# alphanumericslab/EpidemicModeling

Hardware: AMD Instinct MI355X
Metric: region-day EKF steps/sec (300 regions x 400 days x 250 costs) (higher is better)
Workload: dtype f64; 1 GPU; cfg4: SIAlphaModelEKFOptControlled sweep, 300 regions x 250 cost weights x (400+120) days; chains_per_gpu=75000, days=520, outputs=all, storage=f64, spinup_passes=14, lane_block=40, sweep_chains_total=75000, region_day_steps_per_pass_per_gpu=39000000, historic_only_steps_per_pass_per_gpu=30000000, scoring_tail=True

## Files before the change

epidemicmodeling_amd/_build.py:

```python
from __future__ import annotations

import os
import shutil
import subprocess

HERE = os.path.dirname(os.path.abspath(__file__))
SRC = os.path.join(HERE, "csrc", "epiekf.hip")
DEPS = [SRC, os.path.join(HERE, "csrc", "launch_plan.hpp"), os.path.join(HERE, "csrc", "ekf_device.hpp"), os.path.join(HERE, "csrc", "ekf_sym.hpp"), os.path.join(HERE, "csrc", "ekf_quad.hpp"), os.path.join(HERE, "csrc", "ekf_wave.hpp"), os.path.join(HERE, "csrc", "ekf_hex.hpp"), os.path.join(HERE, "csrc", "ekf_lane6.hpp"),
        os.path.join(HERE, "csrc", "scenario_kernels.hpp"), os.path.join(HERE, "csrc", "rt_expfit.hpp"), os.path.join(HERE, "csrc", "preprocess.hpp"), os.path.join(HERE, "csrc", "nnls.hpp"), os.path.join(HERE, "csrc", "lookahead.hpp"), os.path.join(HERE, "csrc", "rt_window.hpp"), os.path.join(HERE, "csrc", "lasso.hpp"), os.path.join(HERE, "csrc", "ens_summary.hpp"), os.path.join(HERE, "csrc", "ens_score.hpp"), os.path.join(HERE, "csrc", "path_functionals.hpp"), os.path.join(HERE, "csrc", "ar_forecast.hpp"), os.path.join(HERE, "csrc", "two_filter.hpp"), os.path.join(HERE, "csrc", "robust_fit.hpp"), os.path.join(HERE, "csrc", "rate_map.hpp"), os.path.join(HERE, "csrc", "mldivide.hpp"), os.path.join(HERE, "csrc", "svr.hpp"), os.path.join(HERE, "csrc", "loglik.hpp"), os.path.join(HERE, "csrc", "npi_plan.hpp"), os.path.join(HERE, "csrc", "smoother_draws.hpp"), os.path.join(HERE, "csrc", "host_stage.hpp"),
        os.path.join(HERE, "..", "include", "epiekf.h"), os.path.join(HERE, "..", "include", "epiekf_layout.h")]
LIB = os.path.join(HERE, "libepiekf.so")

HIPCC_FLAGS = ["--offload-arch=gfx950", "-O3", "-std=c++17", "-ffp-contract=off", "-fPIC", "-shared"]


def source_hash() -> str:
    import hashlib
    h = hashlib.sha256()
    for d in sorted(DEPS):
        h.update(os.path.basename(d).encode())
        h.update(open(d, "rb").read())
    return h.hexdigest()[:16]


def hipcc() -> str:
    for cand in (shutil.which("hipcc"), "/opt/rocm/bin/hipcc"):
        if cand and os.path.exists(cand):
            return cand
    raise RuntimeError("hipcc not found: libepiekf.so cannot be built")


def is_stale() -> bool:
    if not os.path.exists(LIB):
        return True
    t = os.path.getmtime(LIB)
    return any(os.path.getmtime(d) > t for d in DEPS)


def build_library(force: bool = False, verbose: bool = False) -> str:
    if force or is_stale():
        cmd = [hipcc(), *HIPCC_FLAGS, SRC, "-o", LIB]
        if verbose:
            print(" ".join(cmd))
        subprocess.check_call(cmd)
    return LIB
```

epidemicmodeling_amd/csrc/epiekf.hip:

```cpp
#include <hip/hip_runtime.h>
#include <stdio.h>
#include <stdlib.h>
#include <string.h>
#include <sys/mman.h>
#include <atomic>
#include <condition_variable>
#include <deque>
#include <functional>
#include <mutex>
#include <thread>
#include <tuple>
#include <vector>
#include "ekf_device.hpp"

namespace epi {

struct KArgs {
    int B, T, Sx, Su, n_npi, L, r_mode;
    int q_mode;
    ModelFlags mf;
    const int32_t *x_series, *u_series;
    const double *x, *u, *R_series, *R_scalar, *prm;
    const double *s_init, *Ps_init, *s_final, *Ps_final, *Q;
    double *S_MINUS, *S_PLUS, *P_MINUS, *P_PLUS;
// ... 518 lines not shown
                    mat_mul<M>(PAt, X, J);
                    rank = rk & 0xff;
                    st_cap |= (rk >> 8) & 1;
                    min_rank = rank < min_rank ? rank : min_rank;
                }
            } else {
                mrdivide<M>(PAt, Pm1, J);
            }
        }
        if (a.pinv_rank) a.pinv_rank[lay_scalar(t, lay)] = rank;

        double Sn[M];
        {
            double dv[M];
#pragma unroll
            for (int i = 0; i < M; i++) dv[i] = Ss[i] - Sm1[i];
#pragma unroll
            for (int i = 0; i < M; i++) {
                double acc = J[IXM(i, 0)] * dv[0];
#pragma unroll
                for (int j = 1; j < M; j++) acc = fma(J[IXM(i, j)], dv[j], acc);
                Sn[i] = Sp[i] + acc;
            }
        }
        state_hard_margins<M>(p, Sn);
        {
            double D[M * M], T1[M * M], T2[M * M];
#pragma unroll
            for (int e = 0; e < M * M; e++) D[e] = Pm1[e] - Ps[e];
            mat_mul<M>(J, D, T1);
            mat_mul_bt<M>(T1, J, T2);
#pragma unroll
            for (int e = 0; e < M * M; e++) Ps[e] = Pp[e] - T2[e];
        }
        if (GENERIC) symmetrize<M>(Ps);
#pragma unroll
        for (int i = 0; i < M; i++) Ss[i] = Sn[i];
        store_vec<M>(a.S_SMOOTH, t, lay, Ss);
        store_mat<M>(a.P_SMOOTH, t, lay, Ps);
        if (GENERIC && a.u_opt_smooth) {
            double sn_unused[M];
            nlin_state_update<M, FLIP>(p, a.mf, u_in, Ss, sn_unused);
            store_u(a.u_opt_smooth, a, t, lay, u_in);
        }
    }
    if (a.status) a.status[c] = st_guard | (st_cap << 1) | (min_rank << 8);
}

#include "ekf_sym.hpp"
#include "ekf_quad.hpp"
#include "ekf_wave.hpp"
#include "ekf_hex.hpp"
#include "ekf_lane6.hpp"


__global__ __launch_bounds__(256) void sialpha_sim(const epi_sim_desc d, const int32_t *__restrict__ u_series,
                                                   const double *__restrict__ u, const double *__restrict__ sp,
                                                   const double *__restrict__ z, double *__restrict__ so,
                                                   double *__restrict__ io, double *__restrict__ ao,
                                                   double *__restrict__ J0, double *__restrict__ J1,
                                                   const double *__restrict__ J0_prefix,
                                                   const double *__restrict__ J1_prefix,
                                                   const int32_t *__restrict__ gate)
{
    const int c = blockIdx.x * blockDim.x + threadIdx.x;
    if (c >= d.B) return;
    if (gate && *gate == 0) return;
    const int B = d.B;
    const int su = u_series ? u_series[c] : c;
    SimPrm p;
    double s, i, al;
    load_sim_prm(p, sp, B, c, s, i, al);
    const bool pre = (d.prefix_days > 0) && J0_prefix && J1_prefix;
    double acc0 = pre ? J0_prefix[c] : 0.0, acc1 = pre ? J1_prefix[c] : 0.0;
    const int ublk = (d.u_block <= 0 || d.u_block >= d.Su) ? d.Su : d.u_block;
    const size_t unb = (size_t)(d.Su + ublk - 1) / ublk, ucb = (size_t)su / ublk, ucr = (size_t)su % ublk;
    for (int t = 0; t < d.K; t++) {
        double uk[kNpi];
#pragma unroll
        for (int k = 0; k < kNpi; k++) uk[k] = (k < d.n_npi) ? u[(((size_t)t * unb + ucb) * d.n_npi + k) * ublk + ucr] : 0.0;
        double z1 = 0.0, z2 = 0.0, z3 = 0.0;
        if (d.noise) {
            z1 = z[((size_t)t * 3 + 0) * B + c]; z2 = z[((size_t)t * 3 + 1) * B + c]; z3 = z[((size_t)t * 3 + 2) * B + c];
        }
        sialpha_step(p, uk, z1, z2, z3, s, i, al);
        if (so) so[(size_t)t * B + c] = s;
        if (io) io[(size_t)t * B + c] = i;
        if (ao) ao[(size_t)t * B + c] = al;
        if (d.with_cost) npicost_accumulate(p, uk, d.n_npi, t == 0 && !pre, s, i, al, acc0, acc1);
    }
    if (d.with_cost) {
        const size_t days = (size_t)d.K + (size_t)(pre ? d.prefix_days : 0);
        if (J0) J0[c] = acc0 / (double)days;
        if (J1) J1[c] = acc1 / (double)((size_t)d.n_npi * days);
    }
}

#include "scenario_kernels.hpp"
#include "rt_expfit.hpp"
#include "preprocess.hpp"
#include "nnls.hpp"
#include "lookahead.hpp"
#include "rt_window.hpp"
#include "lasso.hpp"
#include "ens_summary.hpp"
#include "ens_score.hpp"
// ... 277 lines not shown
    if constexpr (M == 3 && GENERIC) {
        if (p.fwd.kernel == FWD_WAVE3) e = go(ekf_fwd_wave3<FLIP>);
    }
    if constexpr (GENERIC) {
        if (p.fwd.kernel == FWD_SYM) {
            if (v & V_INLINE) e = (v & V_STOR) ? go(ekf_fwd_sym<M, FLIP, 0, 1>) : (v & V_LP) ? go(ekf_fwd_sym<M, FLIP, 1>) : go(ekf_fwd_sym<M, FLIP, 0>);
            else if (v & V_STOR) e = go(ekf_fwd_sym<M, FLIP, 0, 1, 0>);
            else if (v & V_USD) e = go(ekf_fwd_sym<M, FLIP, 1, 0, 0, 1>);
            else e = (v & V_LP) ? go(ekf_fwd_sym<M, FLIP, 1, 0, 0>) : go(ekf_fwd_sym<M, FLIP, 0, 0, 0>);
        }
    }
    if (e == hipSuccess && p.dense) e = launch(ekf_fwd<M, FLIP, GENERIC>, dim3(o.dense_grid), kWave, p.dense_lds, st, ka);
    return e;
}

template <int M>
static hipError_t enqueue_pinv(KArgs ka, const PlanOp &o, hipStream_t st)
{
    ka.c0 = o.c0; ka.cn = o.cn; ka.pinv_step0 = o.a;
    const dim3 grid(o.grid, (unsigned)o.b);
    return ka.only ? launch(eks_pinv<M, 1>, grid, pinv_wg<M>(), 0, st, ka) : launch(eks_pinv<M, 0>, grid, pinv_wg<M>(), 0, st, ka);
}

template <int M, int FLIP, int GENERIC>
static hipError_t enqueue_bwd(KArgs ka, const LaunchPlan &p, const PlanOp &o, hipStream_t st)
{
    ka.bk_from = o.a; ka.bk_to = o.b; ka.c0 = o.c0; ka.cn = o.cn;
    const unsigned v = p.bwd.bits;
    auto go = [&](auto kern) { return launch(kern, dim3(o.grid), kWave, 0, st, ka, (const int *)ka.dense_flag); };
    hipError_t e = hipSuccess;
    if constexpr (M == 6 && !GENERIC) {
        if (p.bwd.kernel == BWD_WAVE_NC) e = launch(eks_bwd_wave_nc, dim3(o.grid), kWave, 0, st, ka);
    }
    if constexpr (M == 6 && GENERIC) {
        if (p.bwd.kernel == BWD_WAVE) e = go(eks_bwd_wave<FLIP>);
        if (p.bwd.kernel == BWD_HEX)
            e = (v & V_BLK) ? ((v & V_SOLO) ? go(eks_bwd_hex<FLIP, kHG, 2>) : go(eks_bwd_hex<FLIP, kHG, 0>))
                            : ((v & V_SOLO) ? go(eks_bwd_hex<FLIP, 0, 1>) : go(eks_bwd_hex<FLIP, 0, 0>));
        if (p.bwd.kernel == BWD_QUAD) e = (v & V_BLK) ? go(eks_bwd_quad<FLIP, kQC>) : go(eks_bwd_quad<FLIP, 0>);
        if (p.bwd.kernel == BWD_LANE6)
            e = p.bwd.wg_chains == 40 ? (o.xd ? go(eks_bwd_lane6<FLIP, 40, 1>) : go(eks_bwd_lane6<FLIP, 40, 0>))
                                      : (p.bwd.wg_chains == 48 ? go(eks_bwd_lane6<FLIP, 48, 0>) : go(eks_bwd_lane6<FLIP, 56, 0>));
    }
    if constexpr (M == 3 && GENERIC) {
        if (p.bwd.kernel == BWD_WAVE3) e = go(eks_bwd_wave3<FLIP>);
    }
    if constexpr (GENERIC) {
        if (p.bwd.kernel == BWD_SYM) e = (v & V_STOR) ? go(eks_bwd_sym<M, FLIP, 1>) : go(eks_bwd_sym<M, FLIP>);
    }
    if (e == hipSuccess && p.dense) e = launch(eks_bwd<M, FLIP, GENERIC>, dim3(o.dense_grid), kWave, 0, st, ka);
    return e;
}

static hipError_t enqueue_tail(const KArgs &ka, const Tail &t, hipStream_t st, const int32_t *gate = nullptr)
{
    epi_sim_desc sd{};
    sd.abi_version = EPIEKF_ABI_VERSION; sd.B = ka.B; sd.K = ka.T - t.t_hist; sd.Su = ka.B; sd.n_npi = ka.n_npi;
    sd.noise = 0; sd.with_cost = 1; sd.prefix_days = t.t_hist; sd.u_block = ka.blk >= ka.B ? 0 : ka.blk;
    const double *u_h = ka.u_opt_smooth + (size_t)t.t_hist * ka.n_npi * ((size_t)ka.nblk * ka.blk);
    hipLaunchKernelGGL(sialpha_sim, dim3((ka.B + 255) / 256), dim3(256), 0, st, sd, (const int32_t *)nullptr, u_h, t.sp,
                       (const double *)nullptr, (double *)nullptr, (double *)nullptr, (double *)nullptr, t.J0, t.J1,
                       t.J0_prefix, t.J1_prefix, gate);
    hipError_t e = hipGetLastError();
    if (e != hipSuccess || (!t.on_front && !t.i_opt)) return e;
    hipLaunchKernelGGL(pareto_front, dim3(t.R), dim3(256), (size_t)2 * t.P * sizeof(double), st, t.P, t.J0, t.J1, t.on_front, t.i_opt, gate);
    return hipGetLastError();
}

template <int M, int FLIP, int GENERIC>
static hipError_t run_plan(const KArgs &ka, const LaunchPlan &p, const Tail *tail, hipStream_t st, Helper *h)
{
    if (p.overflow || (p.helper && !h)) return hipErrorInvalidValue;
    for (int i = 0; i < p.n_ops; i++) {
        const PlanOp &o = p.ops[i];
        hipStream_t s = o.stream == ON_HELPER ? h->stream : st;
        hipError_t e = hipSuccess;
        switch (o.kind) {
        case OP_FWD: e = enqueue_fwd<M, FLIP, GENERIC>(ka, p, o, s); break;
        case OP_PINV: e = enqueue_pinv<M>(ka, o, s); break;
        case OP_BWD: e = enqueue_bwd<M, FLIP, GENERIC>(ka, p, o, s); break;
        case OP_MONITOR: e = launch_monitor<FLIP>(ka, p, s); break;
        case OP_TAIL: e = enqueue_tail(ka, *tail, s); break;
        case OP_RECORD: e = hipEventRecord(h->ev[o.a], s); break;
        case OP_WAIT: e = hipStreamWaitEvent(s, h->ev[o.a], 0); break;
        }
        if (e != hipSuccess) return e;
    }
    return hipSuccess;
}

template <int M, int FLIP>
static hipError_t rerun_nonfinite_dense(const KArgs &ka, const PlanIn &in, const Tail *tail, hipStream_t st)
{
    hipError_t e = hipMemsetAsync(ka.only_buf + ka.B, 0, sizeof(int32_t), st);
    if (e != hipSuccess) return e;
    hipLaunchKernelGGL(mark_nonfinite, dim3((ka.B + 255) / 256), dim3(256), 0, st, (const int32_t *)ka.status, ka.only_buf, ka.B);
    if ((e = hipGetLastError()) != hipSuccess) return e;
    PlanIn ind = in;
    ind.hint = 2; ind.only = true; ind.smooth = true; ind.rerun = false; ind.has_tail = false;
    const LaunchPlan pd = plan_launch(ind);
    KArgs kd = ka;
    kd.only = ka.only_buf; kd.dense_flag = nullptr; kd.quad = pd.quad; kd.hex = pd.hex; kd.mon_hoist = pd.mon_hoist;
    if ((e = run_plan<M, FLIP, 1>(kd, pd, nullptr, st, nullptr)) != hipSuccess) return e;
    if (tail) e = enqueue_tail(ka, *tail, st, ka.only_buf + ka.B);
    return e;
}

template <int M, int FLIP, int GENERIC>
static hipError_t launch_chain(const KArgs &ka, const PlanIn &in, const LaunchPlan &p, const Tail *tail, int dev, hipStream_t st)
{
    hipError_t e = hipSuccess;
    if (p.precheck >= 0) {
        if ((e = hipMemsetAsync(ka.dense_flag, 0, sizeof(int), st)) != hipSuccess) return e;
        if (p.precheck == 1) hipLaunchKernelGGL((ekf_precheck<M>), dim3((ka.B + 255) / 256), dim3(256), 0, st, ka, ka.dense_flag, 0);
        if (p.precheck == 2) hipLaunchKernelGGL((ekf_precheck<M>), dim3(1), dim3(64), 0, st, ka, ka.dense_flag, 1);
        if ((e = hipGetLastError()) != hipSuccess) return e;
    }
    HelperLease lease(dev);
    if (p.helper) {
        hipStreamCaptureStatus cs = hipStreamCaptureStatusNone;
        if (hipStreamIsCapturing(st, &cs) != hipSuccess) (void)hipGetLastError();
        lease.captured = cs != hipStreamCaptureStatusNone;
        if ((e = helper_acquire(dev, &lease.h)) != hipSuccess) return e;
    }
    e = run_plan<M, FLIP, GENERIC>(ka, p, tail, st, lease.h);
    if constexpr (GENERIC) {
        if (e == hipSuccess && p.rerun_after) e = rerun_nonfinite_dense<M, FLIP>(ka, in, tail, st);
    }
    return e;
}

static PlanIn plan_input(const epi_batch_desc *d, int dev) { PlanIn in{}; in.d = d; in.n_simds = simd_count(dev); return in; }

// ... 4 lines not shown
extern "C" {

int epi_abi_version(void) { return EPIEKF_ABI_VERSION; }

const char *epi_status_string(int status)
{
    switch (status) {
    case EPI_OK: return "ok";
    case EPI_ERR_UNDEFINED_ORDER: return "Undefined order";
    case EPI_ERR_Q_MISMATCH: return "Process noise covariance noise mismatch";
    case EPI_ERR_R_MISMATCH: return "Observation noise covariance noise mismatch";
    case EPI_ERR_OBS_TYPE: return "unknown observation type";
    case EPI_ERR_BAD_ARG: return "bad argument";
    case EPI_ERR_WORKSPACE: return "workspace too small";
    case EPI_ERR_HIP: return "HIP runtime error";
    case EPI_ERR_UNSUPPORTED: return "unsupported";
    default: return "unknown status";
    }
}

int epi_model_dim(int model) { return (model >= 0 && model < 6) ? MODEL_TABLE[model].m : -1; }

int epi_ekf_validate(const epi_batch_desc *d, char *err)
{
    if (!d) { set_err(err, "NULL descriptor"); return EPI_ERR_BAD_ARG; }
    if (d->abi_version != EPIEKF_ABI_VERSION) { set_err(err, "ABI version mismatch"); return EPI_ERR_BAD_ARG; }
    if (d->model < 0 || d->model > 5) { set_err(err, "unknown model"); return EPI_ERR_BAD_ARG; }
    if (d->B < 1 || d->T < 1 || d->Sx < 1 || d->Su < 1 || d->L < 1) { set_err(err, "B, T, Sx, Su, L must be >= 1"); return EPI_ERR_BAD_ARG; }
    if (d->T > 65536) { set_err(err, "T is limited to 65536 (grid y dimension of eks_pinv)"); return EPI_ERR_BAD_ARG; }
    if (d->B > (1 << 23) || d->Sx > (1 << 23) || d->Su > (1 << 23)) { set_err(err, "B, Sx, Su are limited to 2^23 (a per-step array slice is addressed through one 4 GiB buffer descriptor)"); return EPI_ERR_BAD_ARG; }
    if (d->n_npi < 1 || d->n_npi > EPI_MAX_NPI) { set_err(err, "n_npi out of range 1..12"); return EPI_ERR_BAD_ARG; }
    if (d->order != 1 && d->order != 2) { set_err(err, epi_status_string(EPI_ERR_UNDEFINED_ORDER)); return EPI_ERR_UNDEFINED_ORDER; }
    const ModelInfo &mi = MODEL_TABLE[d->model];
    if (!mi.obs_fixed && d->obs_type != EPI_OBS_NEWCASES && d->obs_type != EPI_OBS_TOTALCASES) {
        set_err(err, epi_status_string(EPI_ERR_OBS_TYPE)); return EPI_ERR_OBS_TYPE;
    }
    if (d->q_mode != 0 && d->q_mode != 1) { set_err(err, epi_status_string(EPI_ERR_Q_MISMATCH)); return EPI_ERR_Q_MISMATCH; }
    if (!mi.generic && d->q_mode != 0) {
        set_err(err, epi_status_string(EPI_ERR_Q_MISMATCH)); return EPI_ERR_Q_MISMATCH;
    }
    if (d->r_mode != 0 && d->r_mode != 1) { set_err(err, epi_status_string(EPI_ERR_R_MISMATCH)); return EPI_ERR_R_MISMATCH; }
    if (!mi.generic && d->r_mode != 0) {
        set_err(err, epi_status_string(EPI_ERR_R_MISMATCH)); return EPI_ERR_R_MISMATCH;
    }
    if (d->phase < 0 || d->phase > 4) { set_err(err, "phase must be 0..4"); return EPI_ERR_BAD_ARG; }
    if (d->path_hint < 0 || d->path_hint > 2) { set_err(err, "path_hint must be 0, 1 or 2"); return EPI_ERR_BAD_ARG; }
    if (d->time_pipe < -1 || d->time_pipe > 1) { set_err(err, "time_pipe must be -1 (off), 0 (auto) or 1 (on)"); return EPI_ERR_BAD_ARG; }
    if (d->lane_block < 0) { set_err(err, "lane_block must be >= 0"); return EPI_ERR_BAD_ARG; }
    if (d->shape < 0 || d->shape > 4) { set_err(err, "shape must be 0 (auto), 1 (one lane per chain), 2 (four lanes per chain), 3 (one wavefront per chain) or 4 (six lanes per chain)"); return EPI_ERR_BAD_ARG; }
    if (d->storage < 0 || d->storage > 1) { set_err(err, "storage must be 0 (fp64) or 1 (fp32)"); return EPI_ERR_BAD_ARG; }
    if (d->exact_nonfinite < -1 || d->exact_nonfinite > 1) { set_err(err, "exact_nonfinite must be 0 (default: on), 1 (on) or -1 (off)"); return EPI_ERR_BAD_ARG; }
    if (d->placement_tries < 0 || d->placement_tries > EPI_PLACEMENT_MAX_TRIES) { set_err(err, "placement_tries must be 0 .. EPI_PLACEMENT_MAX_TRIES"); return EPI_ERR_BAD_ARG; }
    if (d->test_window < 0 || d->test_window == 1) { set_err(err, "test_window must be 0 (production) or >= 2"); return EPI_ERR_BAD_ARG; }
    if (d->test_flags < 0 || d->test_flags > 7) { set_err(err, "test_flags must be 0 (production) .. 7"); return EPI_ERR_BAD_ARG; }
    if (padded_chains(d) > ((size_t)1 << 23)) { set_err(err, "B rounded up to lane_block exceeds 2^23"); return EPI_ERR_BAD_ARG; }
    if ((size_t)3 * d->L * kWave * sizeof(double) > 160u * 1024u) { set_err(err, "inv_monitor_len too large for LDS (max 106)"); return EPI_ERR_UNSUPPORTED; }
    return EPI_OK;
}

size_t epi_ekf_workspace_bytes(const epi_batch_desc *d)
{
    if (epi_ekf_validate(d, nullptr) != EPI_OK) return 0;
    return ws_layout(d).total;
}

int epi_ekf_preferred_lane_block(const epi_batch_desc *d)
{
    epi_batch_desc probe;
    if (!d) return 0;
    probe = *d; probe.lane_block = 0;
    if (epi_ekf_validate(&probe, nullptr) != EPI_OK) return 0;
    const int lw = plan_launch(plan_input(d, current_device())).chains_per_wave;
    return lw < d->B ? lw : d->B;
}

static int run_device_impl(const epi_batch_desc *d, const epi_inputs *in, const epi_outputs *out,
                           void *workspace, size_t workspace_bytes, const Tail *tail, void *stream, char *err)
{
    int rc = epi_ekf_validate(d, err);
    if (rc != EPI_OK) return rc;
    if (!in || !out) { set_err(err, "NULL inputs/outputs"); return EPI_ERR_BAD_ARG; }
    const ModelInfo &mi = MODEL_TABLE[d->model];
    if (!in->x || !in->u || !in->prm || !in->s_init || !in->Ps_init || !in->s_final || !in->Ps_final || !in->Q) {
        set_err(err, "NULL input array"); return EPI_ERR_BAD_ARG;
    }
    if (d->r_mode == 0 && !in->R_scalar) { set_err(err, "r_mode 0 needs R_scalar"); return EPI_ERR_BAD_ARG; }
    if (d->r_mode == 1 && !in->R_series) { set_err(err, "r_mode 1 needs R_series"); return EPI_ERR_BAD_ARG; }
    if (!in->x_series && d->Sx != d->B) { set_err(err, "identity x_series needs Sx == B"); return EPI_ERR_BAD_ARG; }
    if (!in->u_series && d->Su != d->B) { set_err(err, "identity u_series needs Su == B"); return EPI_ERR_BAD_ARG; }
    const WsLayout wl = ws_layout(d);
    if (wl.total > 0 && (!workspace || workspace_bytes < wl.total)) {
        set_err(err, epi_status_string(EPI_ERR_WORKSPACE)); return EPI_ERR_WORKSPACE;
    }
    const bool f32 = d->storage == 1;
    if (f32 && (!mi.generic || d->q_mode != 0 || d->path_hint != 1)) {
        set_err(err, "storage = 1 (fp32) runs the packed kernels of the generic models only: fixed Q_w and path_hint = 1 "
                     "(epi_ekf_precheck_device said the batch qualifies)");
        return EPI_ERR_UNSUPPORTED;
    }
    const uint32_t om = f32 ? 0u : d->out_mask;
    const uint32_t om32 = f32 ? d->out_mask : 0u;
    auto sel = [&](uint32_t bit, double *p) -> double * { return (om & bit) ? p : nullptr; };
    auto sel32 = [&](uint32_t bit, double *p) -> float * { return (om32 & bit) ? (float *)p : nullptr; };
    char *ws = (char *)workspace;
    KArgs ka{};
    ka.B = d->B; ka.T = d->T; ka.Sx = d->Sx; ka.Su = d->Su; ka.n_npi = d->n_npi; ka.L = d->L; ka.r_mode = d->r_mode; ka.q_mode = d->q_mode;
    ka.blk = lane_block_of(d); ka.nblk = (d->B + ka.blk - 1) / ka.blk;
// ... 2726 lines not shown
```

epidemicmodeling_amd/csrc/launch_plan.hpp:

```cpp
#pragma once
#include <stddef.h>
#include <stdint.h>
#include "../../include/epiekf.h"

namespace epi {
struct ModelInfo { int m, flipped, lo_is_zero, phi_ge, obs_clamp, obs_fixed, generic; };
static const ModelInfo MODEL_TABLE[6] = {
     {3, 0, 0, 0, 1, 0, 1},
     {6, 0, 1, 0, 1, 0, 1},
     {3, 1, 1, 0, 1, 0, 1},
     {6, 1, 1, 0, 1, 0, 1},
     {6, 0, 1, 1, 1, 0, 0},
     {6, 0, 1, 1, 0, 1, 0},
};

constexpr int kWave = 64;
constexpr int kQC = kWave / 4;
constexpr int kHG = 10;
constexpr int kW3G = 7;
constexpr int kPipeLanes = 40;
constexpr bool lane6_block(int blk) { return blk == 40 || blk == 48 || blk == 56; }
constexpr int pinv_chains(int m) { return m >= 6 ? 64 : 256; }
constexpr int kMonitorParDays = 8;
constexpr int kMonitorParMaxWaves = 2;
// ... 1 lines not shown
constexpr int kTimeSeg = (int)(sizeof(kTimeCuts) / sizeof(kTimeCuts[0])) - 1;
constexpr int kRpParts = 3;
constexpr int kHelperEvents = 16;
constexpr int kMaxPlanOps = 32;

static inline int lane_block_of(const epi_batch_desc *d) { return (d->lane_block <= 0 || d->lane_block >= d->B) ? d->B : d->lane_block; }

static inline bool monitor_hoisted(const epi_batch_desc *d)
{
    return MODEL_TABLE[d->model].generic && d->r_mode == 1 && d->q_mode == 0 && d->path_hint != 2 &&
           (size_t)4 * d->L * kWave * sizeof(double) <= 64u * 1024u;
}
static inline int shape_of(const epi_batch_desc *d, int n_simds)
{
    const ModelInfo &mi = MODEL_TABLE[d->model];
    if (!mi.generic) {
        const bool ok = mi.m == 6 && !d->storage && d->q_mode == 0 && (size_t)6 * d->L * sizeof(double) <= 48u * 1024u;
        if (d->shape == EPI_SHAPE_WAVE) return ok ? EPI_SHAPE_WAVE : EPI_SHAPE_LANE;
        if (d->shape != EPI_SHAPE_AUTO) return EPI_SHAPE_LANE;
        return (ok && (long)d->B <= (long)n_simds) ? EPI_SHAPE_WAVE : EPI_SHAPE_LANE;
    }
    if (d->storage) return EPI_SHAPE_LANE;
    if (mi.m == 3) {
        const bool ok = monitor_hoisted(d);
        if (d->shape == EPI_SHAPE_WAVE) return ok ? EPI_SHAPE_WAVE : EPI_SHAPE_LANE;
        if (d->shape == EPI_SHAPE_LANE || d->shape == EPI_SHAPE_QUAD || d->shape == EPI_SHAPE_HEX) return EPI_SHAPE_LANE;
        return (ok && d->B <= 2048) ? EPI_SHAPE_WAVE : EPI_SHAPE_LANE;
    }
    const bool hex_ok = monitor_hoisted(d) && (long)d->B <= (1L << 20) && (long)d->n_npi * d->Su <= (1L << 25);
    const bool wave_ok = hex_ok || (mi.generic && d->r_mode == 0 && d->q_mode == 0 && d->path_hint != 2 &&
                                    (size_t)6 * d->L * sizeof(double) <= 48u * 1024u);
    if (d->shape == EPI_SHAPE_WAVE) return wave_ok ? EPI_SHAPE_WAVE : EPI_SHAPE_QUAD;
    if (d->shape == EPI_SHAPE_HEX) return hex_ok ? EPI_SHAPE_HEX : EPI_SHAPE_QUAD;
    if (d->shape == EPI_SHAPE_QUAD || d->shape == EPI_SHAPE_LANE) return d->shape;
    if (wave_ok && (long)d->B <= (hex_ok ? (long)n_simds * 5 / 8 : (long)n_simds)) return EPI_SHAPE_WAVE;
    if (hex_ok && ((long)d->B + kHG - 1) / kHG <= 2 * (long)n_simds) return EPI_SHAPE_HEX;
    return ((long)d->B + kQC - 1) / kQC <= (long)n_simds ? EPI_SHAPE_QUAD : EPI_SHAPE_LANE;
}

static inline int balanced_lanes(int cn, int waves_per_simd, int n_simds)
{
    if (waves_per_simd >= 2) return kWave;
    const long cap = (long)n_simds * waves_per_simd;
    const long w64 = (cn + kWave - 1) / kWave;
    if (w64 <= cap) return kWave;
    const long rounds = (w64 + cap - 1) / cap;
    long lw = (cn + rounds * cap - 1) / (rounds * cap);
    lw = (lw + 7) / 8 * 8;
    return (int)(lw > kWave ? kWave : lw);
}

enum PlanStream { ON_MAIN = 0, ON_HELPER = 1 };
enum FwdKernel { FWD_NONE = 0, FWD_WAVE_NC, FWD_WAVE, FWD_WAVE3, FWD_HEX, FWD_QUAD, FWD_SYM };
enum BwdKernel { BWD_NONE = 0, BWD_WAVE_NC, BWD_WAVE, BWD_WAVE3, BWD_HEX, BWD_QUAD, BWD_LANE6, BWD_SYM };
enum MonKernel { MON_NONE = 0, MON_PAR, MON_SCAN };
enum : unsigned {
    V_L21 = 1u,
    V_BLK = 2u,
    V_SOLO = 4u,
    V_INLINE = 8u,
    V_STOR = 16u,
    V_LP = 32u,
    V_USD = 64u,
};
struct KernelPick { int kernel; unsigned bits; int wg_chains; unsigned lds; };
enum ScheduleBits : unsigned {
    SCHED_OVERLAP = 1u,
    SCHED_TIME_PIPE = 2u,
    SCHED_REVERSE_PIPE = 4u,
    SCHED_FWD_RANGES = 8u,
    SCHED_BWD_ROUNDS = 16u,
    SCHED_BWD_HORIZON = 32u,
};
enum PlanOpKind { OP_FWD, OP_PINV, OP_BWD, OP_MONITOR, OP_TAIL, OP_RECORD, OP_WAIT };
struct PlanOp {
    int kind, stream;
    int a, b;
    int c0, cn;
    unsigned grid, dense_grid;
    int xd;
};
struct PlanIn {
    const epi_batch_desc *d;
    int n_simds;
    bool smooth, rerun;
    int hint, ws_upper;
    bool want_rho, only;
    bool has_tail; int t_hist;
};
static inline PlanIn plan_call_input(const epi_batch_desc *d, int n_simds, bool has_pinv_rank, bool has_status, bool has_tail, int t_hist)
{
    const ModelInfo &mi = MODEL_TABLE[d->model];
    const bool f32 = d->storage == 1;
    const uint32_t sel = d->out_mask, om = f32 ? 0u : d->out_mask;
    PlanIn in{}; in.d = d; in.n_simds = n_simds;
    const bool smooth_sel = (sel & (EPI_OUT_S_SMOOTH | EPI_OUT_P_SMOOTH)) || (mi.generic && (sel & EPI_OUT_U_OPT_SMOOTH)) ||
                            has_pinv_rank || has_status;
    in.rerun = mi.generic && (d->exact_nonfinite > 0 || (d->exact_nonfinite == 0 && smooth_sel)) && d->q_mode == 0 && d->phase == 0 && !f32;
    in.smooth = smooth_sel || in.rerun;
    in.hint = (mi.generic && d->q_mode == 0) ? d->path_hint : 2;
    in.ws_upper = ((om & EPI_OUT_P_MINUS) ? 0 : 1) | ((om & EPI_OUT_P_PLUS) ? 0 : 2);
    in.want_rho = (sel & EPI_OUT_RHO) != 0;
    in.has_tail = has_tail; in.t_hist = has_tail ? t_hist : 0;
    return in;
}
struct LaunchPlan {
    bool overflow;
    int shape, chains_per_wave;
    int lw, quad, wave, hex, mon_hoist;
    unsigned schedule;
    int precheck;
    bool helper, dense;
    KernelPick fwd, bwd, mon;
    unsigned dense_lds, mon_gx, mon_gy;
    bool rerun_after;
    int n_ops, n_events;
    PlanOp ops[kMaxPlanOps];
};

static inline LaunchPlan plan_launch(const PlanIn &in)
{
    const epi_batch_desc *d = in.d;
    const ModelInfo &mi = MODEL_TABLE[d->model];
    const int M = mi.m, B = d->B, T = d->T, L = d->L, phase = d->phase, blk = lane_block_of(d), nblk = (B + blk - 1) / blk;
    const long S = in.n_simds;
    const bool generic = mi.generic != 0, stor = d->storage == 1;
    LaunchPlan p{}; p.shape = shape_of(d, in.n_simds);
    p.lw = balanced_lanes(B, M == 6 ? 1 : 2, in.n_simds); p.wave = p.shape == EPI_SHAPE_WAVE;
    p.quad = !in.only && p.shape == EPI_SHAPE_QUAD; p.hex = !in.only && p.shape == EPI_SHAPE_HEX; p.mon_hoist = !in.only && monitor_hoisted(d);
    p.chains_per_wave = p.shape == EPI_SHAPE_WAVE ? 1 : (p.shape == EPI_SHAPE_HEX ? kHG : (p.shape == EPI_SHAPE_QUAD ? kQC : p.lw));
    const bool lane = !p.wave && !p.quad && !p.hex, hoist = p.mon_hoist != 0;
    p.dense = !generic || in.hint != 1;
    p.dense_lds = (unsigned)((size_t)3 * L * kWave * sizeof(double));
    const unsigned l21 = L == 21 ? V_L21 : 0u, inl = hoist ? 0u : V_INLINE;
    const unsigned win6 = (unsigned)((size_t)6 * L * sizeof(double));
    const long fwd_waves = p.hex ? ((long)B + kHG - 1) / kHG : p.quad ? ((long)B + kQC - 1) / kQC : ((long)B + kWave - 1) / kWave;
    const unsigned solo = fwd_waves <= S ? V_SOLO : 0u;
    const bool lane6_ok = M == 6 && generic && lane && !stor && lane6_block(blk) && (long)blk * nblk <= (1L << 20);
    if (!generic && p.wave && !in.only) {
        p.fwd = {FWD_WAVE_NC, l21, 1, win6};
        p.bwd = {BWD_WAVE_NC, 0u, 1, 0u};
        p.dense = false;
    } else if (generic && in.hint != 2) {
        if (p.wave && M == 6) {
            p.fwd = {FWD_WAVE, inl | l21, 1, hoist ? 0u : win6};
            p.bwd = {BWD_WAVE, 0u, 1, 0u};
        } else if (p.wave) {
            p.fwd = {FWD_WAVE3, 0u, kW3G, 0u};
            p.bwd = {BWD_WAVE3, 0u, kW3G, 0u};
        } else if (p.hex) {
            p.fwd = {FWD_HEX, (blk == kHG ? V_BLK : 0u) | solo, kHG, 0u};
            p.bwd = {BWD_HEX, (blk == kHG ? V_BLK : 0u) | solo, kHG, 0u};
        } else if (p.quad) {
            const unsigned qshm = (unsigned)(((size_t)(hoist ? 0 : 6 * L) + EPI_MAX_NPI) * kQC * sizeof(double));
            p.fwd = {FWD_QUAD, ((blk == kQC && L == 21) ? V_BLK : 0u) | inl | (hoist ? solo : 0u), kQC, qshm};
            p.bwd = {BWD_QUAD, blk == kQC ? V_BLK : 0u, kQC, 0u};
        } else {
            const size_t per_lane = ((size_t)3 * L + 4 * EPI_MAX_NPI) * sizeof(double);
            const bool lp = !stor && M == 6 && p.lw <= kPipeLanes && per_lane * kPipeLanes * 4 <= 160u * 1024u;
            const unsigned lds = hoist ? (lp ? (unsigned)((size_t)4 * EPI_MAX_NPI * kPipeLanes * sizeof(double)) : 0u)
                                       : (lp ? (unsigned)(per_lane * kPipeLanes) : p.dense_lds);
            p.fwd = {FWD_SYM, inl | (stor ? V_STOR : 0u) | (lp ? V_LP : 0u) | (lp && hoist && in.ws_upper == 3 ? V_USD : 0u), p.lw, lds};
            p.bwd = lane6_ok ? KernelPick{BWD_LANE6, 0u, blk, 0u} : KernelPick{BWD_SYM, stor ? V_STOR : 0u, p.lw, 0u};
        }
    }
    const bool mon = hoist && in.want_rho;
    if (mon) {
        const long mb = p.mon_gx = (unsigned)(((long)B + kWave - 1) / kWave);
        if (L == 21 && !((d->test_flags >> 1) & 1) && mb <= kMonitorParMaxWaves * S) {
            p.mon = {MON_PAR, V_L21, kWave, 0u};
            p.mon_gy = (unsigned)((T + kMonitorParDays - 1) / kMonitorParDays);
        } else {
            long nseg = (8 * S + mb - 1) / mb;
            const long max_seg = T / 64 > 1 ? T / 64 : 1;
            nseg = nseg < 1 ? 1 : (nseg > max_seg ? max_seg : nseg);
            p.mon = {MON_SCAN, l21, kWave, (unsigned)((size_t)4 * L * kWave * sizeof(double))};
            p.mon_gy = (unsigned)nseg;
        }
    }
    auto push = [&](int kind, int stream, int a, int b, int c0, int cn) {
        if (p.n_ops >= kMaxPlanOps) { p.overflow = true; return; }
        PlanOp &o = p.ops[p.n_ops++];
        o.kind = kind; o.stream = stream; o.a = a; o.b = b; o.c0 = c0; o.cn = cn;
        if (kind == OP_FWD || kind == OP_BWD) {
            const KernelPick &k = kind == OP_FWD ? p.fwd : p.bwd;
            o.grid = k.kernel ? (unsigned)((cn + k.wg_chains - 1) / k.wg_chains) : 0u;
            o.dense_grid = p.dense ? (unsigned)((cn + p.lw - 1) / p.lw) : 0u;
            o.xd = kind == OP_BWD && k.kernel == BWD_LANE6 && blk == 40 && cn % 40 == 0;
        } else if (kind == OP_PINV) {
            unsigned tiles = (unsigned)((cn + pinv_chains(M) - 1) / pinv_chains(M));
            if (in.only && tiles > 8u) tiles = 8u;
            o.grid = tiles >= 8u ? ((tiles + 7u) & ~7u) : tiles;
        }
    };
    auto fwd = [&](int k0, int k1, int c0, int cn) { push(OP_FWD, ON_MAIN, k0, k1, c0, cn); };
    auto bwd = [&](int from, int to, int c0, int cn) { push(OP_BWD, ON_MAIN, from, to, c0, cn); };
    auto pinv = [&](int s, int j_lo, int j_hi, int c0, int cn) { if (j_hi >= j_lo) push(OP_PINV, s, mi.flipped ? (T - 1 - j_hi) : (j_lo - 1), j_hi - j_lo + 1, c0, cn); };
    auto record = [&](int stream) { push(OP_RECORD, stream, p.n_events, 0, 0, 0); return p.n_events++; };
    auto wait = [&](int stream, int ev) { push(OP_WAIT, stream, ev, 0, 0, 0); };
    auto fork = [&](int from, int to) { wait(to, record(from)); };
    auto finish = [&]() { p.overflow |= p.n_events > kHelperEvents; return p; };
    const bool fwd_phase = phase == 0 || phase == 1;
    p.precheck = (fwd_phase && generic && !in.only) ? (in.hint == 0 ? 1 : (in.hint == 2 ? 2 : 0)) : -1;
    if (!(generic && phase == 0 && in.smooth && in.hint == 1)) {
        if (fwd_phase) fwd(0, T, 0, B);
        if (fwd_phase && mon) push(OP_MONITOR, ON_MAIN, 0, 0, 0, B);
        if (!in.smooth) return finish();
        if (generic && (phase == 0 || phase == 2 || phase == 3)) pinv(ON_MAIN, 1, T - 1, 0, B);
        if (phase == 0 || phase == 2 || phase == 4) bwd(T - 2, 0, 0, B);
        if (phase == 0 && in.has_tail) push(OP_TAIL, ON_MAIN, 0, 0, 0, B);
        p.rerun_after = generic && in.rerun && phase == 0 && in.hint != 2;
        return finish();
    }
    p.schedule = SCHED_OVERLAP; p.helper = true;
    const bool tail_cut = in.has_tail && in.t_hist >= 1 && in.t_hist <= T - 2;
    const bool force_split = (d->test_flags >> 2) & 1;
    const bool force_rp = (d->test_flags & 1) && p.hex && hoist && T >= 4 && d->time_pipe >= 0;
    const bool tp = !force_rp && hoist && !stor && T >= 128 && d->time_pipe >= 0 &&
                    (d->time_pipe == 1 || (!p.wave && fwd_waves * 4 <= S * 3));
    const bool rp = force_rp || (!tp && p.hex && hoist && T >= 128 && d->time_pipe >= 0);
    bool helper_busy = false;
    if (rp) {
        p.schedule |= SCHED_REVERSE_PIPE;
        fwd(0, T, 0, B); fork(ON_MAIN, ON_HELPER);
        int seg_hi[1 + kRpParts], seg_lo[1 + kRpParts], ev_pinv[1 + kRpParts] = {}, ns = 0, tail_seg = -1, top = T - 2;
        if (tail_cut) { seg_hi[ns] = top; seg_lo[ns] = in.t_hist; tail_seg = ns++; top = in.t_hist - 1; }
        const int parts = (top + 1 >= 96 || (force_rp && top + 1 >= 6)) ? kRpParts : 1;
        for (int q = 0; q < parts; q++) {
            const int lo = (int)((long)(top + 1) * (parts - 1 - q) / parts);
            seg_hi[ns] = top; seg_lo[ns] = lo; ns++;
            top = lo - 1;
        }
        for (int s = 0; s < ns; s++) {
            pinv(s == 0 ? ON_MAIN : ON_HELPER, seg_lo[s] + 1, seg_hi[s] + 1, 0, B);
            if (s > 0) ev_pinv[s] = record(ON_HELPER);
        }
        for (int s = 0; s < ns; s++) {
            if (s > 0) wait(ON_MAIN, ev_pinv[s]);
            bwd(seg_hi[s], seg_lo[s], 0, B);
            if (s == tail_seg) {
                p.schedule |= SCHED_BWD_HORIZON;
                fork(ON_MAIN, ON_HELPER);
                push(OP_TAIL, ON_HELPER, 0, 0, 0, B);
            }
        }
        if (in.has_tail && tail_seg < 0) push(OP_TAIL, ON_MAIN, 0, 0, 0, B);
        if (mon) push(OP_MONITOR, ON_HELPER, 0, 0, 0, B);
        helper_busy = true;
    } else {
        const long waves = ((long)B + p.lw - 1) / p.lw;
        const long cA = force_split ? (waves / 2) * p.lw : S * p.lw;
        const bool fwd_ranges = M == 6 && lane && cA > 0 && cA < B && (force_split || (p.lw < kWave && in.ws_upper != 3));
        if (tp) {
            p.schedule |= SCHED_TIME_PIPE;
            for (int sg = 0; sg < kTimeSeg; sg++) {
                const int k0 = (int)((long)T * kTimeCuts[sg] / 100);
                const int k1 = (sg == kTimeSeg - 1) ? T : (int)((long)T * kTimeCuts[sg + 1] / 100);
                if (k1 <= k0) continue;
                fwd(k0, k1, 0, B);
                fork(ON_MAIN, ON_HELPER);
                pinv(ON_HELPER, k0 + 1, k1 < T ? k1 : T - 1, 0, B);
            }
// ... 45 lines not shown
```

Baseline: 2.667 billion region-day EKF steps/s.

## Add lane-blocked DMA-prefetching backward smoother kernel for non-generic 6-state path

Adds a new backward RTS smoother kernel for the non-generic M=6 case. It uses the lane-blocked layout with per-lane LDS copies of the control parameters. When the chain count is a multiple of the block, it asynchronously DMAs the next day's filtered state and covariance into LDS while the current step computes, with a hand-counted vmcnt wait. The planner selects it when the forward pass would need more waves than there are SMs (or under a test flag), replacing the previous dense or wave backward kernel. The risks are correctness of the manual waitcnt encoding and that the selection condition may not match this workload's configuration.

```diff
diff --git a/epidemicmodeling_amd/_build.py b/epidemicmodeling_amd/_build.py
--- a/epidemicmodeling_amd/_build.py
+++ b/epidemicmodeling_amd/_build.py
@@ -6,7 +6,7 @@
 
 HERE = os.path.dirname(os.path.abspath(__file__))
 SRC = os.path.join(HERE, "csrc", "epiekf.hip")
-DEPS = [SRC, os.path.join(HERE, "csrc", "launch_plan.hpp"), os.path.join(HERE, "csrc", "ekf_device.hpp"), os.path.join(HERE, "csrc", "ekf_sym.hpp"), os.path.join(HERE, "csrc", "ekf_quad.hpp"), os.path.join(HERE, "csrc", "ekf_wave.hpp"), os.path.join(HERE, "csrc", "ekf_hex.hpp"), os.path.join(HERE, "csrc", "ekf_lane6.hpp"),
+DEPS = [SRC, os.path.join(HERE, "csrc", "launch_plan.hpp"), os.path.join(HERE, "csrc", "ekf_device.hpp"), os.path.join(HERE, "csrc", "ekf_sym.hpp"), os.path.join(HERE, "csrc", "ekf_quad.hpp"), os.path.join(HERE, "csrc", "ekf_wave.hpp"), os.path.join(HERE, "csrc", "ekf_hex.hpp"), os.path.join(HERE, "csrc", "ekf_lane6.hpp"), os.path.join(HERE, "csrc", "ekf_nclane.hpp"),
         os.path.join(HERE, "csrc", "scenario_kernels.hpp"), os.path.join(HERE, "csrc", "rt_expfit.hpp"), os.path.join(HERE, "csrc", "preprocess.hpp"), os.path.join(HERE, "csrc", "nnls.hpp"), os.path.join(HERE, "csrc", "lookahead.hpp"), os.path.join(HERE, "csrc", "rt_window.hpp"), os.path.join(HERE, "csrc", "lasso.hpp"), os.path.join(HERE, "csrc", "ens_summary.hpp"), os.path.join(HERE, "csrc", "ens_score.hpp"), os.path.join(HERE, "csrc", "path_functionals.hpp"), os.path.join(HERE, "csrc", "ar_forecast.hpp"), os.path.join(HERE, "csrc", "two_filter.hpp"), os.path.join(HERE, "csrc", "robust_fit.hpp"), os.path.join(HERE, "csrc", "rate_map.hpp"), os.path.join(HERE, "csrc", "mldivide.hpp"), os.path.join(HERE, "csrc", "svr.hpp"), os.path.join(HERE, "csrc", "loglik.hpp"), os.path.join(HERE, "csrc", "npi_plan.hpp"), os.path.join(HERE, "csrc", "smoother_draws.hpp"), os.path.join(HERE, "csrc", "host_stage.hpp"),
         os.path.join(HERE, "..", "include", "epiekf.h"), os.path.join(HERE, "..", "include", "epiekf_layout.h")]
 LIB = os.path.join(HERE, "libepiekf.so")
diff --git a/epidemicmodeling_amd/csrc/ekf_nclane.hpp b/epidemicmodeling_amd/csrc/ekf_nclane.hpp
--- /dev/null
+++ b/epidemicmodeling_amd/csrc/ekf_nclane.hpp
@@ -0,0 +1,194 @@
+#pragma once
+
+constexpr int kNcStoresBehindDma = 1 + 6 + 36;
+constexpr int nc_vmcnt(int n) { return ((n >> 4) & 3) << 14 | 0x0F70 | (n & 15); }
+static_assert(kNcStoresBehindDma == 43 && kNcStoresBehindDma < 64 && nc_vmcnt(kNcStoresBehindDma) == 0x8F7B && nc_vmcnt(63) == 0xCF7F,
+              "the wait ahead of the image's reads counts the step's stores");
+
+template <int BLK, int XD>
+__global__ __launch_bounds__(kWave) void nclane_eks_bwd(const KArgs a)
+{
+    constexpr int M = 6, IMG = M + M * M;
+    __shared__ __attribute__((aligned(16))) double s_img[XD ? IMG * BLK : 2];
+    __shared__ double vlds[4 * kNpi * BLK];
+    const unsigned img_base = (unsigned)(uintptr_t)(lds_ptr_t)s_img;
+    const int lane = threadIdx.x;
+    const int c = a.c0 + blockIdx.x * BLK + lane;
+    if (lane >= BLK || c >= a.c0 + a.cn) return;
+    const int B = a.B, T = a.T;
+    const int su = a.u_series ? a.u_series[c] : c;
+    const unsigned bp = (unsigned)a.blk * (unsigned)a.nblk;
+    const LwLane ll = lw_lane<BLK>((unsigned)c, (unsigned)a.n_npi);
+    LitePrm<VecLdsT<BLK>> p;
+    load_lite(p, a.prm, B, c, a.mf.lo_is_zero);
+    p.v.base = vlds + lane;
+#pragma unroll
+    for (int k = 0; k < kNpi; k++) {
+        vlds[(0 * kNpi + k) * BLK + lane] = a.prm[(size_t)(EPI_PRM_A + k) * B + c];
+        vlds[(1 * kNpi + k) * BLK + lane] = a.prm[(size_t)(EPI_PRM_U_MIN + k) * B + c];
+        vlds[(2 * kNpi + k) * BLK + lane] = a.prm[(size_t)(EPI_PRM_U_MAX + k) * B + c];
+        vlds[(3 * kNpi + k) * BLK + lane] = a.prm[(size_t)(EPI_PRM_W_EFF + k) * B + c];
+    }
+
+    rsrc_t rSp, rPp, rSm, rPm, rSs, rPs, rPr;
+    int tw = 0;
+    auto rebase = [&](int t0) __attribute__((always_inline)) {
+        tw = t0;
+        const size_t bpl = bp;
+        rSp = lw_rsrc(lw_rebase(a.S_PLUS, t0, 6 * bpl)); rPp = lw_rsrc(lw_rebase(a.P_PLUS, t0, 36 * bpl));
+        rSm = lw_rsrc(lw_rebase(a.S_MINUS, t0, 6 * bpl)); rPm = lw_rsrc(lw_rebase(a.P_MINUS, t0, 36 * bpl));
+        rSs = lw_rsrc(lw_rebase(a.S_SMOOTH, t0, 6 * bpl)); rPs = lw_rsrc(lw_rebase(a.P_SMOOTH, t0, 36 * bpl));
+        rPr = lw_rsrc(lw_rebase(a.pinv_rank, t0, bpl));
+    };
+    auto st_results = [&](const LwDay &d, const double (&S)[M], const double (&P)[M * M]) __attribute__((always_inline)) {
+        __builtin_amdgcn_raw_buffer_store_b32(-1, rPr, ll.v1w, d.o1w, 0);
+#pragma unroll
+        for (int i = 0; i < M; i++) lw_st<BLK>(rSs, ll.v6, d.o6, i, S[i]);
+#pragma unroll
+        for (int e = 0; e < M * M; e++) lw_st<BLK>(rPs, ll.v36, d.o36, e, P[e]);
+    };
+    auto ld_plus = [&](const LwDay &d, double (&S)[M], double (&P)[M * M]) __attribute__((always_inline)) {
+#pragma unroll
+        for (int i = 0; i < M; i++) S[i] = lw_ld<BLK>(rSp, ll.v6, d.o6, i);
+#pragma unroll
+        for (int e = 0; e < M * M; e++) P[e] = lw_ld<BLK>(rPp, ll.v36, d.o36, e);
+    };
+    const unsigned cb = (unsigned)c / (unsigned)BLK;
+    const unsigned vds = cb * 6u * BLK * 8u + (unsigned)lane * 16u, vdp = cb * 36u * BLK * 8u + (unsigned)lane * 16u;
+    auto dma_plus = [&](const LwDay &d) __attribute__((always_inline)) {
+#pragma unroll
+        for (int i = 0; i < M / 2; i++) lw_dma16(rSp, img_base + (unsigned)(2 * i * BLK * 8), vds, d.o6 + (unsigned)(2 * i * BLK * 8));
+#pragma unroll
+        for (int i = 0; i < M * M / 2; i++)
+            lw_dma16(rPp, img_base + (unsigned)((M + 2 * i) * BLK * 8), vdp, d.o36 + (unsigned)(2 * i * BLK * 8));
+    };
+
+    const LwDay ds = lw_stride(a, bp);
+    double Ss[M], Ps[M * M];
+    auto terminal = [&]() __attribute__((always_inline)) {
+        const LwDay dT = lw_day(ds, T - 1 - tw);
+        ld_plus(dT, Ss, Ps);
+#pragma unroll
+        for (int i = 0; i < M; i++) {
+            const double f = a.s_final[(size_t)i * B + c];
+            if (!is_nan(f)) Ss[i] = f;
+        }
+        {
+            double Pf[M * M];
+#pragma unroll
+            for (int e = 0; e < M * M; e++) Pf[e] = a.Ps_final[(size_t)e * B + c];
+            bool rows[M], cols[M];
+#pragma unroll
+            for (int i = 0; i < M; i++) { rows[i] = false; cols[i] = false; }
+#pragma unroll
+            for (int j = 0; j < M; j++)
+#pragma unroll
+                for (int i = 0; i < M; i++)
+                    if (!is_nan(Pf[IXM(i, j)])) { rows[i] = true; cols[j] = true; }
+#pragma unroll
+            for (int j = 0; j < M; j++)
+#pragma unroll
+                for (int i = 0; i < M; i++)
+                    if (rows[i] && cols[j]) Ps[IXM(i, j)] = Pf[IXM(i, j)];
+        }
+        st_results(dT, Ss, Ps);
+    };
+
+    double u_cur[kNpi];
+    auto step = [&](int k, const LwDay &d0) __attribute__((always_inline)) {
+        double Sp[M], Pp[M * M];
+        load_u(a, k, su, u_cur);
+        if (XD) {
+            __builtin_amdgcn_s_waitcnt(nc_vmcnt(kNcStoresBehindDma));
+#pragma unroll
+            for (int i = 0; i < M; i++) Sp[i] = s_img[i * BLK + lane];
+#pragma unroll
+            for (int e = 0; e < M * M; e++) Pp[e] = s_img[(M + e) * BLK + lane];
+            if (k > 0) {
+                __builtin_amdgcn_s_waitcnt(0xc07f);
+                lw_phase();
+                dma_plus(lw_next<-1>(d0, ds));
+            }
+            lw_phase();
+        } else {
+            ld_plus(d0, Sp, Pp);
+        }
+
+        double J[M * M], Sm1[M], Pm1[M * M], D[M * M], dv[M];
+        {
+            const LwDay d1 = lw_next<1>(d0, ds);
+#pragma unroll
+            for (int i = 0; i < M; i++) Sm1[i] = lw_ld<BLK>(rSm, ll.v6, d1.o6, i);
+#pragma unroll
+            for (int e = 0; e < M * M; e++) Pm1[e] = lw_ld<BLK>(rPm, ll.v36, d1.o36, e);
+        }
+        {
+            double A[M * M], PAt[M * M];
+            const bool wave_free = lw_wave_has_free_control(u_cur);
+            jacobian_entries<M, 0>(p, Sp, wave_free ? slope_term<M, 0>(p, u_cur, Sp) : 0.0, A);
+            mat_mul_bt<M>(Pp, A, PAt);
+#pragma unroll
+            for (int e = 0; e < M * M; e++) D[e] = Pm1[e] - Ps[e];
+#pragma unroll
+            for (int i = 0; i < M; i++) dv[i] = Ss[i] - Sm1[i];
+            lw_phase();
+            mrdivide<M>(PAt, Pm1, J);
+        }
+
+        double Sn[M];
+        {
+#pragma unroll
+            for (int i = 0; i < M; i++) {
+                double acc = J[IXM(i, 0)] * dv[0];
+#pragma unroll
+                for (int j = 1; j < M; j++) acc = fma(J[IXM(i, j)], dv[j], acc);
+                Sn[i] = Sp[i] + acc;
+            }
+        }
+        state_hard_margins<M>(p, Sn);
+#pragma unroll
+        for (int i = 0; i < M; i++) {
+            double T1r[M];
+#pragma unroll
+            for (int j = 0; j < M; j++) {
+                double acc = J[IXM(i, 0)] * D[IXM(0, j)];
+#pragma unroll
+                for (int q = 1; q < M; q++) acc = fma(J[IXM(i, q)], D[IXM(q, j)], acc);
+                T1r[j] = acc;
+            }
+#pragma unroll
+            for (int j = 0; j < M; j++) {
+                double acc = T1r[0] * J[IXM(j, 0)];
+#pragma unroll
+                for (int q = 1; q < M; q++) acc = fma(T1r[q], J[IXM(j, q)], acc);
+                Ps[IXM(i, j)] = Pp[IXM(i, j)] - acc;
+            }
+        }
+#pragma unroll
+        for (int i = 0; i < M; i++) Ss[i] = Sn[i];
+        lw_phase();
+        st_results(d0, Ss, Ps);
+        lw_phase();
+    };
+
+    const int W = lw_window(a, bp);
+    const auto window_base = [&](int hi) { return hi >= W ? hi - W : 0; };
+    rebase(T >= 2 ? window_base(T - 2) : 0);
+    terminal();
+    if (T >= 2) {
+        if (XD) dma_plus(lw_day(ds, T - 2 - tw));
+    }
+    __builtin_amdgcn_s_waitcnt(0);
+    lw_phase();
+    int k = T - 2;
+    while (k >= 0) {
+        const int hi = k, lo = (hi >= W) ? hi - W + 1 : 0;
+        rebase(window_base(hi));
+        LwDay d0 = lw_day(ds, hi - tw);
+        for (; k >= lo; k--) {
+            step(k, d0);
+            d0 = lw_next<-1>(d0, ds);
+        }
+    }
+    if (a.status) a.status[c] = M << 8;
+}
diff --git a/epidemicmodeling_amd/csrc/epiekf.hip b/epidemicmodeling_amd/csrc/epiekf.hip
--- a/epidemicmodeling_amd/csrc/epiekf.hip
+++ b/epidemicmodeling_amd/csrc/epiekf.hip
@@ -594,6 +594,7 @@
 #include "ekf_wave.hpp"
 #include "ekf_hex.hpp"
 #include "ekf_lane6.hpp"
+#include "ekf_nclane.hpp"
 
 
 __global__ __launch_bounds__(256) void sialpha_sim(const epi_sim_desc d, const int32_t *__restrict__ u_series,
@@ -977,6 +978,22 @@
     return e;
 }
 
+template <int M, int GENERIC>
+static hipError_t enqueue_bwd_nc(KArgs ka, const LaunchPlan &p, const PlanOp &o, hipStream_t st)
+{
+    if constexpr (M == 6 && !GENERIC) {
+        ka.c0 = o.c0; ka.cn = o.cn;
+        auto go = [&](auto kern) { return launch(kern, dim3(o.grid), kWave, 0, st, ka); };
+        if (p.bwd.kernel != BWD_NCLANE) return hipErrorInvalidValue;
+        switch (p.bwd.wg_chains) {
+        case 40: return o.xd ? go(nclane_eks_bwd<40, 1>) : go(nclane_eks_bwd<40, 0>);
+        case 48: return o.xd ? go(nclane_eks_bwd<48, 1>) : go(nclane_eks_bwd<48, 0>);
+        case 56: return o.xd ? go(nclane_eks_bwd<56, 1>) : go(nclane_eks_bwd<56, 0>);
+        }
+    }
+    return hipErrorInvalidValue;
+}
+
 static hipError_t enqueue_tail(const KArgs &ka, const Tail &t, hipStream_t st, const int32_t *gate = nullptr)
 {
     epi_sim_desc sd{};
@@ -1004,6 +1021,7 @@
         case OP_FWD: e = enqueue_fwd<M, FLIP, GENERIC>(ka, p, o, s); break;
         case OP_PINV: e = enqueue_pinv<M>(ka, o, s); break;
         case OP_BWD: e = enqueue_bwd<M, FLIP, GENERIC>(ka, p, o, s); break;
+        case OP_BWD_NC: e = enqueue_bwd_nc<M, GENERIC>(ka, p, o, s); break;
         case OP_MONITOR: e = launch_monitor<FLIP>(ka, p, s); break;
         case OP_TAIL: e = enqueue_tail(ka, *tail, s); break;
         case OP_RECORD: e = hipEventRecord(h->ev[o.a], s); break;
@@ -1114,7 +1132,7 @@
     if (d->exact_nonfinite < -1 || d->exact_nonfinite > 1) { set_err(err, "exact_nonfinite must be 0 (default: on), 1 (on) or -1 (off)"); return EPI_ERR_BAD_ARG; }
     if (d->placement_tries < 0 || d->placement_tries > EPI_PLACEMENT_MAX_TRIES) { set_err(err, "placement_tries must be 0 .. EPI_PLACEMENT_MAX_TRIES"); return EPI_ERR_BAD_ARG; }
     if (d->test_window < 0 || d->test_window == 1) { set_err(err, "test_window must be 0 (production) or >= 2"); return EPI_ERR_BAD_ARG; }
-    if (d->test_flags < 0 || d->test_flags > 7) { set_err(err, "test_flags must be 0 (production) .. 7"); return EPI_ERR_BAD_ARG; }
+    if (d->test_flags < 0 || d->test_flags > 15) { set_err(err, "test_flags must be 0 (production) .. 15"); return EPI_ERR_BAD_ARG; }
     if (padded_chains(d) > ((size_t)1 << 23)) { set_err(err, "B rounded up to lane_block exceeds 2^23"); return EPI_ERR_BAD_ARG; }
     if ((size_t)3 * d->L * kWave * sizeof(double) > 160u * 1024u) { set_err(err, "inv_monitor_len too large for LDS (max 106)"); return EPI_ERR_UNSUPPORTED; }
     return EPI_OK;
diff --git a/epidemicmodeling_amd/csrc/launch_plan.hpp b/epidemicmodeling_amd/csrc/launch_plan.hpp
--- a/epidemicmodeling_amd/csrc/launch_plan.hpp
+++ b/epidemicmodeling_amd/csrc/launch_plan.hpp
@@ -77,7 +77,7 @@
 
 enum PlanStream { ON_MAIN = 0, ON_HELPER = 1 };
 enum FwdKernel { FWD_NONE = 0, FWD_WAVE_NC, FWD_WAVE, FWD_WAVE3, FWD_HEX, FWD_QUAD, FWD_SYM };
-enum BwdKernel { BWD_NONE = 0, BWD_WAVE_NC, BWD_WAVE, BWD_WAVE3, BWD_HEX, BWD_QUAD, BWD_LANE6, BWD_SYM };
+enum BwdKernel { BWD_NONE = 0, BWD_WAVE_NC, BWD_WAVE, BWD_WAVE3, BWD_HEX, BWD_QUAD, BWD_LANE6, BWD_SYM, BWD_NCLANE };
 enum MonKernel { MON_NONE = 0, MON_PAR, MON_SCAN };
 enum : unsigned {
     V_L21 = 1u,
@@ -97,7 +97,7 @@
     SCHED_BWD_ROUNDS = 16u,
     SCHED_BWD_HORIZON = 32u,
 };
-enum PlanOpKind { OP_FWD, OP_PINV, OP_BWD, OP_MONITOR, OP_TAIL, OP_RECORD, OP_WAIT };
+enum PlanOpKind { OP_FWD, OP_PINV, OP_BWD, OP_MONITOR, OP_TAIL, OP_RECORD, OP_WAIT, OP_BWD_NC };
 struct PlanOp {
     int kind, stream;
     int a, b;
@@ -162,10 +162,14 @@
     const long fwd_waves = p.hex ? ((long)B + kHG - 1) / kHG : p.quad ? ((long)B + kQC - 1) / kQC : ((long)B + kWave - 1) / kWave;
     const unsigned solo = fwd_waves <= S ? V_SOLO : 0u;
     const bool lane6_ok = M == 6 && generic && lane && !stor && lane6_block(blk) && (long)blk * nblk <= (1L << 20);
+    const bool nclane_ok = !generic && M == 6 && lane && !in.only && !stor && d->q_mode == 0 && lane6_block(blk) &&
+                           (long)blk * nblk <= (1L << 20) && (((d->test_flags >> 3) & 1) || fwd_waves > S);
     if (!generic && p.wave && !in.only) {
         p.fwd = {FWD_WAVE_NC, l21, 1, win6};
         p.bwd = {BWD_WAVE_NC, 0u, 1, 0u};
         p.dense = false;
+    } else if (nclane_ok) {
+        p.bwd = {BWD_NCLANE, 0u, blk, 0u};
     } else if (generic && in.hint != 2) {
         if (p.wave && M == 6) {
             p.fwd = {FWD_WAVE, inl | l21, 1, hoist ? 0u : win6};
@@ -212,6 +216,9 @@
             o.grid = k.kernel ? (unsigned)((cn + k.wg_chains - 1) / k.wg_chains) : 0u;
             o.dense_grid = p.dense ? (unsigned)((cn + p.lw - 1) / p.lw) : 0u;
             o.xd = kind == OP_BWD && k.kernel == BWD_LANE6 && blk == 40 && cn % 40 == 0;
+        } else if (kind == OP_BWD_NC) {
+            o.grid = (unsigned)((cn + blk - 1) / blk);
+            o.xd = cn % blk == 0;
         } else if (kind == OP_PINV) {
             unsigned tiles = (unsigned)((cn + pinv_chains(M) - 1) / pinv_chains(M));
             if (in.only && tiles > 8u) tiles = 8u;
@@ -232,7 +239,11 @@
         if (fwd_phase && mon) push(OP_MONITOR, ON_MAIN, 0, 0, 0, B);
         if (!in.smooth) return finish();
         if (generic && (phase == 0 || phase == 2 || phase == 3)) pinv(ON_MAIN, 1, T - 1, 0, B);
-        if (phase == 0 || phase == 2 || phase == 4) bwd(T - 2, 0, 0, B);
+        if ((phase == 0 || phase == 2 || phase == 4) && p.bwd.kernel == BWD_NCLANE) {
+            const int cA = (((d->test_flags >> 2) & 1) && nblk >= 2) ? (nblk / 2) * blk : B;
+            push(OP_BWD_NC, ON_MAIN, T - 2, 0, 0, cA);
+            if (cA < B) push(OP_BWD_NC, ON_MAIN, T - 2, 0, cA, B - cA);
+        } else if (phase == 0 || phase == 2 || phase == 4) bwd(T - 2, 0, 0, B);
         if (phase == 0 && in.has_tail) push(OP_TAIL, ON_MAIN, 0, 0, 0, B);
         p.rerun_after = generic && in.rerun && phase == 0 && in.hint != 2;
         return finish();
```

Result: slower. 2.634 billion region-day EKF steps/s (-1.2%).
